# youssefg7/dl-sound-classification

Measured on AMD Instinct MI355X. Metric: training clips/sec (EnvNet-v2, ESC-50 shape), higher is better.
Workload: dtype bf16; 1 GPU; EnvNet-v2 train step (BC-mix, fwd, soft-CE, bwd, clip, Adam), ESC-50 shape; global_batch=256, per_gpu_batch=256, clip_samples=220500, parallelism=dp1, model=envnet_v2

## Files before the change

### dl-sound-classification_amd/csrc/feconv.hip

```cpp
#include "common.h"

#include <type_traits>

namespace {

constexpr int F1_DEPTH = 4;
constexpr int FE_NT = 256;
constexpr int FE_BM = 128;
constexpr int FE_N = 64;

typedef unsigned u32x4 __attribute__((ext_vector_type(4)));

template <int CIN, int KW, int S>
struct FeCfg {
  static constexpr int CG = CIN / 8;
  static constexpr int WPX = (FE_BM - 1) * S + KW;
  static constexpr int HALF = (WPX + 1) / 2;
  static constexpr int NSLOT = S == 1 ? WPX : 2 * HALF;
  static constexpr int PSB = CIN * 2 + 16;
  static constexpr int WBYTES = NSLOT * PSB;
  static constexpr int NCH = WPX * CG;
  static constexpr int LCH = (NCH + FE_NT - 1) / FE_NT;
  static constexpr int KS = KW * CIN / 16;
  static_assert(FE_NT % CG == 0, "channel chunk must be constant per thread");
  static_assert(KS == 32, "weights-in-registers layout assumes K = 512");
};

struct FeArgs {
  const bf16* x;
  const float* ps;
  const float* pt;
  const bf16* w;
  const float* bias;
// ... 180 lines not shown
    if (blockIdx.x < 64 && kst < 256 && lane == 0) {
#pragma unroll
      for (int k = 0; k < 8; ++k) g_fe_st[(((int)blockIdx.x * 4 + wave) * 256 + kst) * 8 + k] = ts[k];
    }
    ++kst;
#endif
  };

  int item = blockIdx.x;
  load(item, rawa, oka);
  load(item + (int)gridDim.x, rawb, okb);
  __syncthreads();
  store(0, rawa, oka);
  __syncthreads();
  for (;;) {
    step(item, 0, rawa, oka, rawb, okb);
    item += gridDim.x;
    if (item >= items) break;
    step(item, 1, rawb, okb, rawa, oka);
    item += gridDim.x;
    if (item >= items) break;
  }
}

constexpr int FS_NT = 512;
#ifndef FS_DEPTH
#define FS_DEPTH 3
#endif
#ifndef FS_FD
#define FS_FD 4
#endif


template <int CIN, int KW, int S, bool PRE>
__global__ __launch_bounds__(FS_NT) __attribute__((amdgpu_waves_per_eu(2, 2))) void feconv_ws_kernel(FeArgs g) {
  using Cfg = FeCfg<CIN, KW, S>;
  __shared__ __attribute__((aligned(16))) char smem[2 * Cfg::WBYTES];
  __shared__ __attribute__((aligned(16))) float sbias[FE_N];
  __shared__ __attribute__((aligned(16))) float spre[2][CIN];
  const int t = threadIdx.x, lane = t & 63, wave = t >> 6;
  const int items = g.n * g.nitem;
  if ((int)blockIdx.x >= items) return;
  const int nk = (items - 1 - (int)blockIdx.x) / (int)gridDim.x + 1;
  if (t < FE_N) sbias[t] = g.bias ? g.bias[t] : 0.f;
  if (PRE && t < CIN) {
    spre[0][t] = g.ps[t];
    spre[1][t] = g.pt[t];
  }
  if (wave < 4) {
    const int nh = wave & 1, pq = wave >> 1;
    bf16x8 wf[Cfg::KS];
    {
      const bf16* wr = g.w + (int64_t)(nh * 32 + (lane & 31)) * (KW * CIN) + 8 * (lane >> 5);
#pragma unroll
      for (int ks = 0; ks < Cfg::KS; ++ks) wf[ks] = *reinterpret_cast<const bf16x8*>(wr + ks * 16);
    }
    const int c0 = nh * 32 + 8 * (lane >> 5);
    lds_barrier();
    lds_barrier();
#pragma unroll 1
    for (int k = 0; k < nk; ++k) {
      const int item = (int)blockIdx.x + k * (int)gridDim.x;
      f32x16 acc[2];
#pragma unroll
      for (int i = 0; i < 2; ++i)
#pragma unroll
        for (int r = 0; r < 16; ++r) acc[i][r] = 0.f;
      const char* win = smem + (k & 1) * Cfg::WBYTES;
      auto frag = [&](int ks, int i) __attribute__((always_inline)) {
        constexpr int KPC = CIN / 16;
        const int kx = ks / KPC;
        const int ci = (ks % KPC) * 16 + 8 * (lane >> 5);
        const int px = pq * 64 + i * 32 + (lane & 31);
        int slot;
        if constexpr (S == 1) slot = px + kx;
        else slot = (kx & 1) * Cfg::HALF + px + (kx >> 1);
        return *reinterpret_cast<const bf16x8*>(win + slot * Cfg::PSB + ci * 2);
      };
#ifdef FS_PROBE_NOCOMPUTE
      if (g.n < 0)
#endif
      {
        bf16x8 fr[FS_FD][2];
#pragma unroll
        for (int ks = 0; ks < FS_FD; ++ks)
#pragma unroll
          for (int i = 0; i < 2; ++i) fr[ks][i] = frag(ks, i);
#pragma unroll
        for (int ks = 0; ks < Cfg::KS; ++ks) {
#pragma unroll
          for (int i = 0; i < 2; ++i) {
            acc[i] = __builtin_amdgcn_mfma_f32_32x32x16_bf16(wf[ks], fr[ks % FS_FD][i], acc[i], 0, 0, 0);
            if (ks + FS_FD < Cfg::KS) fr[ks % FS_FD][i] = frag(ks + FS_FD, i);
          }
        }
        __builtin_amdgcn_sched_group_barrier(0x100, 2 * FS_FD, 0);
#pragma unroll
        for (int ks = 0; ks < Cfg::KS; ++ks) {
          __builtin_amdgcn_sched_group_barrier(0x008, 2, 0);
          if (ks + FS_FD < Cfg::KS) __builtin_amdgcn_sched_group_barrier(0x100, 2, 0);
        }
      }
      const int b = item / g.nitem;
      const int m0 = (item - b * g.nitem) * FE_BM + pq * 64;
      bf16* yb = g.y + (int64_t)b * g.ystride;
#pragma unroll
      for (int i = 0; i < 2; ++i) {
        float v[16];
#pragma unroll
        for (int h = 0; h < 2; ++h)
#pragma unroll
          for (int j = 0; j < 4; ++j) {
            const float lo = acc[i][8 * h + j], hi = acc[i][8 * h + 4 + j];
            const auto r = __builtin_amdgcn_permlane32_swap(__float_as_uint(lo), __float_as_uint(hi), false, false);
            v[8 * h + j] = __builtin_bit_cast(float, (unsigned)r[0]);
            v[8 * h + 4 + j] = __builtin_bit_cast(float, (unsigned)r[1]);
          }
        const int m = m0 + i * 32 + (lane & 31);
        if (m < g.wout) {
#pragma unroll
          for (int h = 0; h < 2; ++h) {
            const int64_t e = (int64_t)m * FE_N + c0 + 16 * h;
            if (e < g.ylen) {
              const f32x4 u0 = *reinterpret_cast<const f32x4*>(sbias + c0 + 16 * h);
              const f32x4 u1 = *reinterpret_cast<const f32x4*>(sbias + c0 + 16 * h + 4);
              const u32x4 o = {pack2(v[8 * h] + u0[0], v[8 * h + 1] + u0[1]), pack2(v[8 * h + 2] + u0[2], v[8 * h + 3] + u0[3]),
                               pack2(v[8 * h + 4] + u1[0], v[8 * h + 5] + u1[1]), pack2(v[8 * h + 6] + u1[2], v[8 * h + 7] + u1[3])};
              *reinterpret_cast<u32x4*>(yb + e) = o;
            }
          }
        }
      }
      lds_barrier();
    }
  } else {
    const int ft = t - 256;
    const int cg = ft % Cfg::CG;
    const __amdgpu_buffer_rsrc_t xr = __builtin_amdgcn_make_buffer_rsrc(
        const_cast<bf16*>(g.x), (short)0, (int)((int64_t)g.n * g.win * CIN * 2), 0x00020000);
    auto load = [&](int k, u32x4 (&raw)[Cfg::LCH], uint32_t& rok) __attribute__((always_inline)) {
      int it = (int)blockIdx.x + k * (int)gridDim.x;
      it = it < items ? it : items - 1;
      const int b = it / g.nitem;
      const int px0 = (it - b * g.nitem) * FE_BM * S - g.pw;
      rok = 0;
#pragma unroll
      for (int s = 0; s < Cfg::LCH; ++s) {
        const int q = ft + FE_NT * s;
        const int p = q / Cfg::CG;
        const int ix = px0 + p;
        const bool ok = p < Cfg::WPX && ix >= 0 && ix < g.win;
        const unsigned off = ok ? (unsigned)((b * g.win + ix) * Cfg::CG + cg) * 16u : 0x80000000u;
#ifdef FS_PROBE_NOLOAD
        raw[s] = u32x4{0u, 0u, 0u, 0u};
        (void)off;
#else
        raw[s] = __builtin_bit_cast(u32x4, __builtin_amdgcn_raw_buffer_load_b128(xr, off, 0, 0));
#endif
        rok |= (uint32_t)ok << s;
      }
    };
    auto stage = [&](int buf, const u32x4 (&raw)[Cfg::LCH], uint32_t rok) __attribute__((always_inline)) {
      float sc[8], sh[8];
      if constexpr (PRE) {
#pragma unroll
        for (int h = 0; h < 2; ++h) {
// ... 12 lines not shown
              fe_cook(raw[s], (rok >> s) & 1u, PRE, sc, sh);
      }
    };
    u32x4 raw[FS_DEPTH][Cfg::LCH];
    uint32_t rok[FS_DEPTH];
#pragma unroll
    for (int d = 0; d < FS_DEPTH; ++d) load(d, raw[d], rok[d]);
    lds_barrier();
    stage(0, raw[0], rok[0]);
    lds_barrier();
    static_assert(12 % FS_DEPTH == 0, "feeder unroll");
    auto iter = [&](auto KC, int k) __attribute__((always_inline)) {
      constexpr int R = decltype(KC)::value;
      constexpr int SET = R % FS_DEPTH, NXT = (R + 1) % FS_DEPTH;
      load(k + FS_DEPTH, raw[SET], rok[SET]);
      if (k + 1 < nk) stage((R + 1) & 1, raw[NXT], rok[NXT]);
      lds_barrier();
    };
    auto step = [&](auto KC, int k) __attribute__((always_inline)) {
      const int kk = k + decltype(KC)::value;
      if (kk < nk) iter(KC, kk);
      return kk + 1 < nk;
    };
#pragma unroll 1
    for (int k = 0; k < nk; k += 12) {
      using std::integral_constant;
      (void)(step(integral_constant<int, 0>{}, k) && step(integral_constant<int, 1>{}, k) &&
             step(integral_constant<int, 2>{}, k) && step(integral_constant<int, 3>{}, k) &&
             step(integral_constant<int, 4>{}, k) && step(integral_constant<int, 5>{}, k) &&
             step(integral_constant<int, 6>{}, k) && step(integral_constant<int, 7>{}, k) &&
             step(integral_constant<int, 8>{}, k) && step(integral_constant<int, 9>{}, k) &&
             step(integral_constant<int, 10>{}, k) && step(integral_constant<int, 11>{}, k));
    }
  }
}

struct F1Args {
  const float* x;
  const bf16* w;
  const float* bias;
  bf16* y;
  float* part;
  int n, t, w1, nitem;
};

template <bool STATS>
__global__ __launch_bounds__(256) void fe_conv1_kernel(F1Args g) {
  __shared__ __attribute__((aligned(16))) uint32_t seg[4][160];
  __shared__ __attribute__((aligned(16))) char stage[4][2048];
  const int lane = threadIdx.x & 63, wv = threadIdx.x >> 6;
  const int gw = blockIdx.x * 4 + wv, nw = gridDim.x * 4;
  const int items = g.n * g.nitem;
  uint32_t* sg = seg[wv];
  bf16x8 wa[4];
#pragma unroll
  for (int ks = 0; ks < 4; ++ks) wa[ks] = *reinterpret_cast<const bf16x8*>(g.w + (lane & 31) * 64 + ks * 16 + 8 * (lane >> 5));
  const int c0 = 8 * (lane >> 5);
  float bv[16];
#pragma unroll
  for (int i = 0; i < 8; ++i) { bv[i] = g.bias[c0 + i]; bv[8 + i] = g.bias[c0 + 16 + i]; }
  float s1[16], s2[16];
#pragma unroll
  for (int i = 0; i < 16; ++i) { s1[i] = 0.f; s2[i] = 0.f; }

  typedef float f32x2 __attribute__((ext_vector_type(2)));
  auto load = [&](int it) __attribute__((always_inline)) {
// ... 512 lines not shown
bool reduce_v1() { const char* e = getenv("MIA_REDUCE_V1"); return e && e[0] == '1'; }

bool aligned16(const void* p) { return (reinterpret_cast<uintptr_t>(p) & 15) == 0; }

bool fe_ws() { const char* e = getenv("MIA_FECONV_WS"); return !(e && e[0] == '0'); }

}

extern "C" int mia_fe_conv2_fwd(const void* y1, const float* scale, const float* shift, const void* w,
                                const float* bias, void* y2, int32_t n, int32_t w1, int32_t w2,
                                mia_stream_t stream) {
  MIA_CHECK_ARG(y1 && w && y2 && n > 0 && w1 >= 16, "fe_conv2_fwd: bad arguments");
  MIA_CHECK_ARG(!scale == !shift, "fe_conv2_fwd: scale and shift go together");
  MIA_CHECK_ARG(w2 == (w1 - 16) / 2 + 1, "fe_conv2_fwd: w2 must be (w1-16)/2+1 (got w1=%d w2=%d)", w1, w2);
  MIA_CHECK_ARG(aligned16(y1) && aligned16(w) && aligned16(y2), "fe_conv2_fwd: operands must be 16-byte aligned");
  hipStream_t s = as_stream(stream);
  const int per = fe_clips_per_launch((int64_t)w1 * 32 * 2);
  MIA_CHECK_ARG(per > 0, "fe_conv2_fwd: one clip exceeds 2 GB");
  for (int c = 0; c < n; c += per) {
    const int nc = n - c < per ? n - c : per;
    FeArgs a{reinterpret_cast<const bf16*>(y1) + (int64_t)c * w1 * 32, scale, shift, reinterpret_cast<const bf16*>(w),
             bias, reinterpret_cast<bf16*>(y2) + (int64_t)c * w2 * FE_N, nc, w1, w2, 0, (int)cdiv(w2, FE_BM),
             (int64_t)w2 * FE_N, (int64_t)w2 * FE_N};
    if (fe_ws()) {
      const int grid = fe_grid1(nc * a.nitem);
      if (scale) feconv_ws_kernel<32, 16, 2, true><<<grid, FS_NT, 0, s>>>(a);
      else feconv_ws_kernel<32, 16, 2, false><<<grid, FS_NT, 0, s>>>(a);
    } else {
      const int grid = fe_grid(nc * a.nitem);
      if (scale) feconv_kernel<32, 16, 2, true><<<grid, FE_NT, 0, s>>>(a);
      else feconv_kernel<32, 16, 2, false><<<grid, FE_NT, 0, s>>>(a);
    }
    MIA_LAUNCH_CHECK("fe_conv2_fwd");
  }
  return 0;
}

extern "C" int mia_fe_conv2_dgrad(const void* dy2, const void* wpar, void* da1, int32_t n, int32_t w1,
                                  int32_t w2, mia_stream_t stream) {
  MIA_CHECK_ARG(dy2 && wpar && da1 && n > 0 && w1 >= 16, "fe_conv2_dgrad: bad arguments");
  MIA_CHECK_ARG(w2 == (w1 - 16) / 2 + 1, "fe_conv2_dgrad: w2 must be (w1-16)/2+1 (got w1=%d w2=%d)", w1, w2);
  MIA_CHECK_ARG(aligned16(dy2) && aligned16(wpar) && aligned16(da1), "fe_conv2_dgrad: operands must be 16-byte aligned");
  MIA_CHECK_ARG(((int64_t)w1 * 32) % 8 == 0, "fe_conv2_dgrad: clip stride must keep 16-byte alignment");
  const int wout = (w1 + 1) / 2;
  const int per = fe_clips_per_launch((int64_t)w2 * 64 * 2);
  MIA_CHECK_ARG(per > 0, "fe_conv2_dgrad: one clip exceeds 2 GB");
  for (int c = 0; c < n; c += per) {
    const int nc = n - c < per ? n - c : per;
    FeArgs a{reinterpret_cast<const bf16*>(dy2) + (int64_t)c * w2 * 64, nullptr, nullptr,
             reinterpret_cast<const bf16*>(wpar), nullptr, reinterpret_cast<bf16*>(da1) + (int64_t)c * w1 * 32, nc,
             w2, wout, 7, (int)cdiv(wout, FE_BM), (int64_t)w1 * 32, (int64_t)w1 * 32};
#ifdef FS_DGRAD
    feconv_ws_kernel<64, 8, 1, false><<<fe_grid1(nc * a.nitem), FS_NT, 0, as_stream(stream)>>>(a);
#else
    feconv_kernel<64, 8, 1, false><<<fe_grid(nc * a.nitem), FE_NT, 0, as_stream(stream)>>>(a);
#endif
    MIA_LAUNCH_CHECK("fe_conv2_dgrad");
  }
  return 0;
}

extern "C" int mia_fe_conv2_wgrad(const void* dy2, const void* y1, const float* scale, const float* shift,
                                  float* dw, int32_t n, int32_t w1, int32_t w2, void* workspace, int64_t ws_bytes,
                                  mia_stream_t stream) {
  MIA_CHECK_ARG(dy2 && y1 && dw && workspace && n > 0 && w1 >= 16, "fe_conv2_wgrad: bad arguments");
  MIA_CHECK_ARG(!scale == !shift, "fe_conv2_wgrad: scale and shift go together");
// ... 65 lines not shown
```

### dl-sound-classification_amd/src/miaudio/kernels.py

```python
from __future__ import annotations

import math
from dataclasses import dataclass

import os

import torch

from . import lib as L

_WS: dict = {}


def workspace(nbytes: int, device, slot: str = "main") -> torch.Tensor:
    key = (str(device), slot)
    buf = _WS.get(key)
    nbytes = max(int(nbytes), 256)
    if buf is None or buf.numel() < nbytes:
        buf = torch.empty(int(nbytes * 1.25) + 256, dtype=torch.uint8, device=device)
        _WS[key] = buf
    return buf


def _s():
# ... 463 lines not shown
    assert dw.dtype == torch.float32 and dw.numel() == 32 * 64 and dbias.dtype == torch.float32 and dbias.numel() == 32
    nw = 4096
    lib = L.load()
    part = workspace(int(lib.mia_conv3_wgrad_workspace_bytes(nw)), x.device, "conv3w")
    with probe(tag or "", 2.0 * n * oh * ow * 32 * 64, x.numel() * 2 + da.numel() * 6):
        L.check(lib.mia_conv3_wgrad_bn(x.data_ptr(), da.data_ptr(), ya.data_ptr(), dy.data_ptr(), dw.data_ptr(),
                                       dbias.data_ptr(), part.data_ptr(), nw, n, h, wd, L.ptr(gamma),
                                       bn.scale.data_ptr(), bn.shift.data_ptr(), bn.mean.data_ptr(),
                                       bn.invstd.data_ptr(), dgamma.data_ptr(), dbeta.data_ptr(), _s()),
                "mia_conv3_wgrad_bn")


def bn_finalize_shifted(partial: torch.Tensor, nblk: int, P: int, C: int, kshift: torch.Tensor, gamma, beta,
                        running_mean, running_var, momentum: float, eps: float) -> BNState:
    st = torch.empty(4, C, dtype=torch.float32, device=partial.device)
    L.check(L.load().mia_bn_finalize_shifted(partial.data_ptr(), nblk, P, C, kshift.data_ptr(), L.ptr(gamma),
                                             L.ptr(beta), L.ptr(running_mean), L.ptr(running_var), momentum, eps, 1,
                                             st[0].data_ptr(), st[1].data_ptr(), st[2].data_ptr(), st[3].data_ptr(),
                                             _s()), "mia_bn_finalize_shifted")
    return BNState(st[0], st[1], st[2], st[3])


def fe_conv2_fwd(y1: torch.Tensor, scale, shift, w: torch.Tensor, bias, y2: torch.Tensor, n: int, w1: int,
                 w2: int, tag: str | None = None):
    assert y1.dtype == torch.bfloat16 and y2.dtype == torch.bfloat16 and w.dtype == torch.bfloat16
    assert y1.numel() == n * w1 * 32 and y2.numel() == n * w2 * 64 and w.numel() == 64 * 512
    assert y1.is_contiguous() and y2.is_contiguous() and w.is_contiguous()
    flop = 2.0 * n * w2 * 64 * 512
    with probe(tag or "", flop, y1.numel() * 2 + y2.numel() * 2):
        L.check(L.load().mia_fe_conv2_fwd(y1.data_ptr(), L.ptr(scale), L.ptr(shift), w.data_ptr(), L.ptr(bias),
                                          y2.data_ptr(), n, w1, w2, _s()), "mia_fe_conv2_fwd")


def fe_conv2_dgrad(dy2: torch.Tensor, wpar: torch.Tensor, da1: torch.Tensor, n: int, w1: int, w2: int,
                   tag: str | None = None):
    assert dy2.dtype == torch.bfloat16 and da1.dtype == torch.bfloat16 and wpar.dtype == torch.bfloat16
    assert dy2.numel() == n * w2 * 64 and da1.numel() == n * w1 * 32 and wpar.numel() == 64 * 512
    assert dy2.is_contiguous() and da1.is_contiguous() and wpar.is_contiguous()
    flop = 2.0 * n * w1 * 32 * 512
    with probe(tag or "", flop, dy2.numel() * 2 + da1.numel() * 2):
        L.check(L.load().mia_fe_conv2_dgrad(dy2.data_ptr(), wpar.data_ptr(), da1.data_ptr(), n, w1, w2, _s()),
                "mia_fe_conv2_dgrad")


def fe_conv2_wgrad(dy2: torch.Tensor, y1: torch.Tensor, scale, shift, dw: torch.Tensor, n: int, w1: int, w2: int,
                   tag: str | None = None):
    assert dy2.dtype == torch.bfloat16 and y1.dtype == torch.bfloat16 and dw.dtype == torch.float32
    assert dy2.numel() == n * w2 * 64 and y1.numel() == n * w1 * 32 and dw.numel() == 64 * 512
    nlaunch = -(-(n * w1 * 64) // (2 ** 31 - 1)) + 1
    nbytes = 512 * nlaunch * 64 * 512 * 4
    ws = workspace(nbytes, dy2.device, "fw")
    flop = 2.0 * n * w2 * 64 * 512
    with probe(tag or "", flop, (dy2.numel() + y1.numel()) * 2):
        L.check(L.load().mia_fe_conv2_wgrad(dy2.data_ptr(), y1.data_ptr(), L.ptr(scale), L.ptr(shift), dw.data_ptr(),
                                            n, w1, w2, ws.data_ptr(), ws.numel(), _s()), "mia_fe_conv2_wgrad")


def fe_conv1_wgrad_bn(x: torch.Tensor, dact: torch.Tensor, y1: torch.Tensor, n: int, t: int, gamma, bn: BNState,
                      dw: torch.Tensor, dbias: torch.Tensor, tag: str | None = None):
    w1 = (t - 64) // 2 + 1
    assert dact.dtype == torch.bfloat16 and y1.dtype == torch.bfloat16 and x.dtype == torch.float32
    assert dact.numel() == n * w1 * 32 and y1.numel() == n * w1 * 32 and x.numel() == n * t
    assert dw.numel() == 32 * 64 and dw.dtype == torch.float32 and dbias.numel() == 32
    split = 512
    ws = workspace((split * (2 * 2048 + 96) + 2 * 2048 + n * 80 + 2 * 160 + 4) * 4, x.device, "tapw")
    g = torch.empty(2, 32, dtype=torch.float32, device=x.device)
# ... 379 lines not shown
```

### dl-sound-classification_amd/src/miaudio/lib.py

```python
from __future__ import annotations

import ctypes as C
import os
from pathlib import Path

import torch

PKG_ROOT = Path(__file__).resolve().parents[2]
LIB_PATH = Path(os.environ.get("MIAUDIO_LIB") or PKG_ROOT / "lib" / "libmiaudio.so")

F32, BF16, U8 = 0, 1, 2
MXFP8 = 16
OP_DENSE, OP_CONV, OP_CONVROW = 0, 1, 2
KC, RC = 0, 1
PRE_NONE, PRE_AFFINE, PRE_AFFINE_RELU, PRE_GELU = 0, 1, 2, 3
ACT_NONE, ACT_RELU, ACT_GELU, DACT_NZ, DACT_GELU, ACT_ADD_AUX, ACT_GELU_SAVE = 0, 1, 2, 3, 4, 5, 6
ACT_GELU_SAVE_D, DACT_MUL = 7, 8

vp = C.c_void_p
i32 = C.c_int32
i64 = C.c_int64
f32 = C.c_float


# ... 118 lines not shown
    "mia_tokens_bwd": (C.c_int, [vp, vp, vp, vp, i32, i32, i32, vp]),
    "mia_ast_patches": (C.c_int, [vp, i32, i32, i32, i32, i32, vp, vp]),
    "mia_tokens_fwd_inplace": (C.c_int, [vp, vp, vp, i32, i32, i32, vp]),
    "mia_cast": (C.c_int, [vp, i32, vp, i32, i64, vp]),
    "mia_add_inplace": (C.c_int, [vp, vp, i32, i64, vp]),
    "mia_bc_mix": (C.c_int, [vp, vp, i64, i32, vp, vp, vp, vp, i32, vp, vp, vp, vp, vp]),
    "mia_bc_partner": (C.c_int, [vp, i32, vp, i32, vp, vp, vp]),
    "mia_stretch_gain": (C.c_int, [vp, i64, i32, vp, vp, vp, vp]),
    "mia_spec_augment_mixup":(C.c_int, [vp, vp, vp, i32, i32, i32, vp, vp, vp, vp, vp, vp, vp]),
    "mia_leaf_workspace_bytes": (i64, [i32, i64, i32, i32, i32, i32]),
    "mia_leaf_energy_fwd": (C.c_int, [vp, vp, vp, i32, i64, i32, i32, i32, i32, vp, vp]),
    "mia_leaf_energy_bwd": (C.c_int, [vp, vp, vp, vp, i32, i64, i32, i32, i32, i32, vp, vp]),
    "mia_pcen_workspace_bytes": (i64, [i32, i32]),
    "mia_pcen_fwd": (C.c_int, [vp, vp, vp, f32, vp, i32, i32, i32, vp]),
    "mia_pcen_bwd": (C.c_int, [vp, vp, vp, f32, vp, vp, vp, vp, vp, i32, i32, i32, vp]),
    "mia_lt_stats_blocks": (i32, [i32, i32, i32, i32]),
    "mia_lt_workspace_bytes": (i64, [i32]),
    "mia_lt_pool_stats": (C.c_int, [vp, i32, i32, i32, i32, i32, vp, vp, vp, vp, vp, i32, vp]),
    "mia_lt_pool_apply": (C.c_int, [vp, i32, i32, i32, i32, vp, vp, vp, i32, i32, vp]),
    "mia_lt_pool_bwd_gather": (C.c_int, [vp, i32, i32, vp, i32, i32, i32, i32, vp, vp, vp, vp, vp, vp, vp, vp, vp]),
    "mia_lt_pool_bwd_apply": (C.c_int, [vp, vp, vp, i32, i32, i32, i32, i32, vp, vp, vp, vp, vp, vp, vp, vp, vp]),
    "mia_lt_pcen_fwd": (C.c_int, [vp, vp, vp, f32, vp, i32, i32, i32, i32, i32, vp]),
    "mia_lt_pcen_bwd": (C.c_int, [vp, vp, vp, f32, vp, i32, vp, vp, vp, vp, i32, i32, i32, i32, vp]),
    "mia_resample_out_len": (i64, [i64, i32, i32]),
    "mia_resample": (C.c_int, [vp, i64, i32, i64, vp, vp, i32, i32, i32, vp, i64, i64, vp]),
    "mia_clip_sgd": (C.c_int, [vp, vp, vp, vp, vp, i32, i64, i64, f32, f32, f32, f32, i32, f32, vp, vp, vp, vp, vp,
                               vp]),
    "mia_clip_adamw": (C.c_int, [vp, vp, vp, vp, vp, vp, i32, i64, i64, f32, f32, f32, f32, f32, i32, f32, vp, vp, vp,
                                 vp, vp, vp]),
    "mia_gemm_sgd": (C.c_int, [P(MiaOperand), P(MiaOperand), i64, i64, i64, vp, vp, vp, i64, vp, f32, f32, f32, f32,
                               i32, i32, vp]),
    "mia_gemm_adamw": (C.c_int, [P(MiaOperand), P(MiaOperand), i64, i64, i64, vp, vp, vp, vp, i64, vp, f32, f32, f32,
                                 f32, f32, f32, f32, vp]),
    "mia_last_error_string": (C.c_char_p, []),
    "mia_device_arch": (C.c_int, [C.c_char_p, i32]),
}

_LIB = None


def load(path: Path | str | None = None):
    global _LIB
    if _LIB is not None:
        return _LIB
    p = Path(path) if path else LIB_PATH
    if not p.exists():
        raise RuntimeError(f"libmiaudio.so not found at {p}: build it with `make -C {PKG_ROOT}` "
                           "(the MI355X kernels have no CPU fallback)")
    lib = C.CDLL(str(p))
    for name, (res, args) in SIGNATURES.items():
        fn = getattr(lib, name, None)
        if fn is None:
            continue
        fn.restype = res
        fn.argtypes = args
    _LIB = lib
    return lib


def exported_symbols():
    lib = load()
    return {n for n in SIGNATURES if hasattr(lib, n)}


def check(rc: int, what: str):
    if rc != 0:
# ... 37 lines not shown
```

### dl-sound-classification_amd/src/models/envnet_hip.py

```python
from __future__ import annotations

import itertools
import os

import torch

from ..miaudio import kernels as K
from ..miaudio import lib as L

_SEED = itertools.count(0x5EED)
C8_BNSEP = os.environ.get("MIA_C8_BNSEP", "0") == "1"
C3_BNSEP = os.environ.get("MIA_C3_BNSEP", "0") == "1"
FC1_CHUNK_ROWS = 256


def _use_conv8(cd: int, cin: int, cout: int, kh: int, kw: int) -> bool:
    return cd == L.BF16 and cin == 32 and cout == 32 and kh == 8 and kw == 8

TRUNK = [
    (("trunk", 0, 0), ("trunk", 0, 1), 1, 32, 8, 8),
    (("trunk", 0, 3), ("trunk", 0, 4), 32, 32, 8, 8),
    (("trunk", 1, 0), ("trunk", 1, 1), 32, 64, 1, 4),
    (("trunk", 1, 3), ("trunk", 1, 4), 64, 64, 1, 4),
    (("trunk", 2, 0), ("trunk", 2, 1), 64, 128, 1, 2),
    (("trunk", 2, 3), ("trunk", 2, 4), 128, 128, 1, 2),
    (("trunk", 3, 0), ("trunk", 3, 1), 128, 256, 1, 2),
    (("trunk", 3, 3), ("trunk", 3, 4), 256, 256, 1, 2),
]
TRUNK_POOL = [(5, 3), (1, 2), (1, 2), (1, 2)]


def geometry(T: int):
    W1 = (T - 64) // 2 + 1
    W2 = (W1 - 16) // 2 + 1
    Wp = W2 // 64
    g = {"T": T, "W1": W1, "W2": W2, "Wp": Wp, "trunk": []}
    H, W = 64, Wp
    for blk in range(4):
        ka = TRUNK[2 * blk]
        ha, wa = H - ka[4] + 1, W - ka[5] + 1
        kb = TRUNK[2 * blk + 1]
        hb, wb = ha - kb[4] + 1, wa - kb[5] + 1
        ph, pw = TRUNK_POOL[blk]
        g["trunk"].append(((H, W), (ha, wa), (hb, wb), (hb // ph, wb // pw)))
        H, W = hb // ph, wb // pw
    g["flat"] = 256 * H * W
    return g


def _frontend_work(B: int, g: dict, tdt: torch.dtype, backward: bool):
    es = torch.finfo(tdt).bits // 8
    X = g["T"] * 4
    S1 = g["W1"] * 32 * es
    S2 = g["W2"] * 64 * es
    P = 64 * g["Wp"] * es
    flop = 2.0 * (g["W1"] * 32 * 64 + g["W2"] * 64 * 512)
    if backward:
        return B * 2 * flop, B * (P + 4 * S2 + 4 * S1 + X)
    return B * flop, B * (X + 2 * S1 + 2 * S2 + P)


def _param_list(m):
    ps = [m.frontend[0].weight, m.frontend[0].bias, m.frontend[1].weight, m.frontend[1].bias,
          m.frontend[3].weight, m.frontend[3].bias, m.frontend[4].weight, m.frontend[4].bias]
    for blk in range(4):
        seq = m.trunk[blk]
        ps += [seq[0].weight, seq[0].bias, seq[1].weight, seq[1].bias,
               seq[3].weight, seq[3].bias, seq[4].weight, seq[4].bias]
    for idx in (1, 4, 7):
        ps += [m.classifier[idx].weight, m.classifier[idx].bias]
    return ps


def _bns(m):
    out = [m.frontend[1], m.frontend[4]]
    for blk in range(4):
        out += [m.trunk[blk][1], m.trunk[blk][4]]
    return out


class EnvNetFunction(torch.autograd.Function):
    @staticmethod
    def forward(ctx, model, x, compute: int, *params):
        if not x.is_cuda:
            raise RuntimeError("EnvNetV2 runs on the MI355X HIP kernels only (input is on CPU)")
        B = x.shape[0]
        x = x.reshape(B, -1).contiguous().float()
        T = x.shape[1]
        if T % 2:
            raise ValueError(f"EnvNetV2 expects an even clip length (got {T})")
        g = geometry(T)
        if g["flat"] != model.classifier[1].in_features:
            raise ValueError(f"clip length {T} gives {g['flat']} trunk features, FC1 expects "
                             f"{model.classifier[1].in_features} (envnet_v2.py:51)")
        training = model.training
        cd = compute
        tdt = L.torch_dtype(cd)
        dev = x.device
        bns = _bns(model)
        p = params
        W1, W2, Wp = g["W1"], g["W2"], g["Wp"]
        saved = {"g": g, "B": B, "cd": cd}

        def bn(i, y, P, C):
            mod = bns[i]
            return K.bn_fwd_stats(y, P, C, mod.weight, mod.bias, mod.running_mean, mod.running_var,
                                  mod.momentum if mod.momentum is not None else 0.1, mod.eps, training)

        wpk = dict(zip([0, 4] + [8 + 8 * b + o for b in range(4) for o in (0, 4)],
                       K.pack_weights([(p[i], cd, 0) for i in [0, 4] + [8 + 8 * b + o for b in range(4) for o in (0, 4)]])))
        saved["wpk"] = wpk
        fe = K.probe("frontend.fwd", *_frontend_work(B, g, tdt, backward=False))
        fe.__enter__()
        w1 = wpk[0]
        y1 = torch.empty(B * W1, 32, dtype=tdt, device=dev)
        if cd == L.BF16:
            st = K.fe_conv1_fwd(x, w1, p[1], y1, B, T, stats=training, tag="conv1.fwd")
            if training:
                m0 = bns[0]
                bn1 = K.bn_finalize_shifted(st[0], st[1], B * W1, 32, p[1], m0.weight, m0.bias, m0.running_mean,
                                            m0.running_var, m0.momentum if m0.momentum is not None else 0.1, m0.eps)
            else:
                bn1 = bn(0, y1, B * W1, 32)
        else:
            A = K.conv(x, L.KC, B, 1, T // 2, 2, 1, W1, 1, 32, row_kind=True)
            Bo = K.dense(w1, L.KC, 32, 64)
            K.gemm(A, Bo, K.epilogue(y1, 32, bias=p[1]), B * W1, 32, 64, cd, tag="conv1.fwd")
            bn1 = bn(0, y1, B * W1, 32)
        w2 = wpk[4]
        y2 = torch.empty(B * W2, 64, dtype=tdt, device=dev)
        if cd == L.BF16:
            K.fe_conv2_fwd(y1, bn1.scale, bn1.shift, w2, p[5], y2, B, W1, W2, tag="conv2.fwd")
        else:
            A = K.conv(y1, L.KC, B, 1, W1, 32, 1, W2, 1, 16, sw=2, pre=L.PRE_AFFINE_RELU, scale=bn1.scale,
                       shift=bn1.shift)
            K.gemm(A, K.dense(w2, L.KC, 64, 512), K.epilogue(y2, 64, bias=p[5]), B * W2, 64, 512, cd,
                   tag="conv2.fwd")
        X0 = torch.empty(B, 64, Wp, dtype=tdt, device=dev)
        am0 = torch.empty(B, Wp, 64, dtype=torch.uint8, device=dev)
        if cd == L.BF16 and training:
            win0 = torch.empty(B, Wp, 64, dtype=tdt, device=dev)
            part2, nb2 = K.pool_raw_stats(y2, B, 1, W2, 64, 1, 64, p[6], p[5], win0, am0)
            m1 = bns[1]
            bn2 = K.bn_finalize_shifted(part2, nb2, B * W2, 64, p[5], m1.weight, m1.bias, m1.running_mean,
                                        m1.running_var, m1.momentum if m1.momentum is not None else 0.1, m1.eps)
            K.pool_apply(win0, B, 1, Wp, 64, bn2, X0, 1)
        else:
            bn2 = bn(1, y2, B * W2, 64)
            K.pool_fwd(y2, B, 1, W2, 64, 1, 64, bn2, X0, 1, am0)
        fe.__exit__(None, None, None)
        saved.update(x=x, y1=y1, y2=y2, bn1=bn1, bn2=bn2, X0=X0, am0=am0,
                     win0=win0 if cd == L.BF16 and training else None)

        inp = X0
        trunk_saved = []
        for blk in range(4):
            (H, W), (ha, wa), (hb, wb), (hp, wp) = g["trunk"][blk]
            _, _, cin, cout, kh, kw = TRUNK[2 * blk]
            pa = 8 + 8 * blk
            wa_ = wpk[pa]
            ya = torch.empty(B * ha * wa, cout, dtype=tdt, device=dev)
            dense_w2 = cd == L.BF16 and kh == 1 and kw == 2 and cin > 1
            conv3_st = None
            if dense_w2:
                K.conv_w2_fwd(inp.reshape(B * H * W, cin), B * H, W, cin, wa_, p[pa + 1], ya, tag=f"t{blk}a.fwd")
            elif cd == L.BF16 and cin == 1 and kh == 8 and kw == 8 and cout == 32 and W % 4 == 0:
                conv3_st = K.fe_conv3_fwd(inp, wa_, p[pa + 1], ya, B, H, W, stats=training, tag=f"t{blk}a.fwd")
            else:
                if cin == 1:
                    A = K.conv(inp, L.KC, B, H, W, 1, ha, wa, kh, kw, row_kind=True)
                else:
                    A = K.conv(inp, L.KC, B, H, W, cin, ha, wa, kh, kw)
                K.gemm(A, K.dense(wa_, L.KC, cout, kh * kw * cin), K.epilogue(ya, cout, bias=p[pa + 1]),
                       B * ha * wa, cout, kh * kw * cin, cd, tag=f"t{blk}a.fwd")
            if conv3_st is not None:
# ... 302 lines not shown
```

Before: 15260 clips/s.

## Fuse BN statistics and max-pool window selection into conv2 forward epilogue

Adds a POOL variant of the warp-specialized conv2 kernel whose epilogue computes per-channel shifted BN sum/sumsq partials and the sign-aware argmax over each 64-wide pool window, writing the pooled raw value and argmax index directly. The training frontend path uses it by default, skipping the separate pool_raw_stats pass that re-read the conv2 output. In exchange the epilogue gains cross-lane permutes, DPP reductions, an extra barrier and a final LDS reduction, which raises register pressure in a kernel pinned to two waves per EU.

```diff
diff --git a/dl-sound-classification_amd/csrc/feconv.hip b/dl-sound-classification_amd/csrc/feconv.hip
--- a/dl-sound-classification_amd/csrc/feconv.hip
+++ b/dl-sound-classification_amd/csrc/feconv.hip
@@ -1,4 +1,6 @@
 #include "common.h"
+
+#include "../../include/miaudio_frontend.h"
 
 #include <type_traits>
 
@@ -245,12 +247,37 @@
 #endif
 
 
-template <int CIN, int KW, int S, bool PRE>
-__global__ __launch_bounds__(FS_NT) __attribute__((amdgpu_waves_per_eu(2, 2))) void feconv_ws_kernel(FeArgs g) {
+struct FePoolArgs : FeArgs {
+  const float* gamma;
+  uint16_t* pwin;
+  uint8_t* amax;
+  float* part;
+  int wp, slot0, zfrom, nslots;
+};
+
+typedef float f32x2 __attribute__((ext_vector_type(2)));
+typedef short s16x2 __attribute__((ext_vector_type(2)));
+
+__device__ __forceinline__ uint32_t fe_code2(uint32_t k) {
+  const s16x2 a = __builtin_bit_cast(s16x2, k) >> (short)15;
+  const s16x2 x = __builtin_bit_cast(s16x2, k & 0x7fff7fffu) ^ a;
+  return __builtin_bit_cast(uint32_t, (s16x2)(x - a));
+}
+template <int N>
+__device__ __forceinline__ int fe_max_ror(int v) {
+  const int o = __builtin_amdgcn_update_dpp(0, v, 0x120 + N, 0xf, 0xf, true);
+  return o > v ? o : v;
+}
+
+template <int CIN, int KW, int S, bool PRE, bool POOL = false>
+__global__ __launch_bounds__(FS_NT) __attribute__((amdgpu_waves_per_eu(2, 2))) void feconv_ws_kernel(
+    std::conditional_t<POOL, FePoolArgs, FeArgs> g) {
   using Cfg = FeCfg<CIN, KW, S>;
   __shared__ __attribute__((aligned(16))) char smem[2 * Cfg::WBYTES];
   __shared__ __attribute__((aligned(16))) float sbias[FE_N];
   __shared__ __attribute__((aligned(16))) float spre[2][CIN];
+  __shared__ __attribute__((aligned(16))) uint32_t ssgn[FE_N / 2];
+  static_assert(!POOL || 4 * 64 * 33 * 4 <= 2 * Cfg::WBYTES, "statistics image fits the window buffers");
   const int t = threadIdx.x, lane = t & 63, wave = t >> 6;
   const int items = g.n * g.nitem;
   if ((int)blockIdx.x >= items) return;
@@ -260,6 +287,9 @@
     spre[0][t] = g.ps[t];
     spre[1][t] = g.pt[t];
   }
+  if constexpr (POOL) {
+    if (t < FE_N / 2) ssgn[t] = (g.gamma[2 * t] < 0.f ? 0x8000u : 0u) | (g.gamma[2 * t + 1] < 0.f ? 0x80000000u : 0u);
+  }
   if (wave < 4) {
     const int nh = wave & 1, pq = wave >> 1;
     bf16x8 wf[Cfg::KS];
@@ -269,6 +299,19 @@
       for (int ks = 0; ks < Cfg::KS; ++ks) wf[ks] = *reinterpret_cast<const bf16x8*>(wr + ks * 16);
     }
     const int c0 = nh * 32 + 8 * (lane >> 5);
+    const int cb = nh * 32 + 4 * (lane >> 5);
+    const int lch = cb + 2 * (lane & 1) + ((lane >> 4) & 1) + 8 * ((lane >> 1) & 3);
+    const int posf = 63 - (lane & 31);
+    uint32_t lsgn = 0;
+    bool lgz = false;
+    f32x2 s1[8], s2[8];
+    if constexpr (POOL) {
+      const float gv = g.gamma[lch];
+      lsgn = gv < 0.f ? 0x8000u : 0u;
+      lgz = gv == 0.f;
+#pragma unroll
+      for (int pp = 0; pp < 8; ++pp) s1[pp] = s2[pp] = f32x2{0.f, 0.f};
+    }
     lds_barrier();
     lds_barrier();
 #pragma unroll 1
@@ -317,6 +360,102 @@
       const int b = item / g.nitem;
       const int m0 = (item - b * g.nitem) * FE_BM + pq * 64;
       bf16* yb = g.y + (int64_t)b * g.ystride;
+      if constexpr (POOL) {
+#ifndef FS_POOL_LATE_BARRIER
+        lds_barrier();
+#endif
+        float bv[16];
+        uint32_t sg[8];
+#pragma unroll
+        for (int q = 0; q < 4; ++q) {
+          const f32x4 u = *reinterpret_cast<const f32x4*>(sbias + cb + 8 * q);
+          const uint2 m2 = *reinterpret_cast<const uint2*>(ssgn + (cb >> 1) + 4 * q);
+#pragma unroll
+          for (int j = 0; j < 4; ++j) bv[4 * q + j] = u[j];
+          sg[2 * q] = m2.x;
+          sg[2 * q + 1] = m2.y;
+        }
+        uint32_t P[2][8];
+#pragma unroll
+        for (int i = 0; i < 2; ++i)
+#pragma unroll
+          for (int pp = 0; pp < 8; ++pp)
+            P[i][pp] = pack2(acc[i][2 * pp] + bv[2 * pp], acc[i][2 * pp + 1] + bv[2 * pp + 1]);
+        const bool full = m0 + 64 <= g.wout;
+        auto stats = [&](auto MASKED) __attribute__((always_inline)) {
+#pragma unroll
+          for (int i = 0; i < 2; ++i) {
+            const bool ok = m0 + i * 32 + (lane & 31) < g.wout;
+#pragma unroll
+            for (int pp = 0; pp < 8; ++pp) {
+              const f32x2 f = {__uint_as_float(P[i][pp] << 16), __uint_as_float(P[i][pp] & 0xffff0000u)};
+              f32x2 d = f - f32x2{bv[2 * pp], bv[2 * pp + 1]};
+              if constexpr (decltype(MASKED)::value) d = ok ? d : f32x2{0.f, 0.f};
+              s1[pp] += d;
+              s2[pp] = __builtin_elementwise_fma(d, d, s2[pp]);
+            }
+          }
+        };
+        if (full) {
+          stats(std::false_type{});
+          int R[8];
+#pragma unroll
+          for (int pp = 0; pp < 8; ++pp) {
+            const uint32_t c0 = fe_code2(P[0][pp] ^ sg[pp]), c1 = fe_code2(P[1][pp] ^ sg[pp]);
+            const int l0 = (int)((c0 << 16) | (uint32_t)posf), l1 = (int)((c1 << 16) | (uint32_t)(posf - 32));
+            const int h0 = (int)((c0 & 0xffff0000u) | (uint32_t)posf), h1 = (int)((c1 & 0xffff0000u) | (uint32_t)(posf - 32));
+            const int ka = l0 > l1 ? l0 : l1, kb = h0 > h1 ? h0 : h1;
+            const auto sw = __builtin_amdgcn_permlane16_swap((unsigned)ka, (unsigned)kb, false, false);
+            const int u0 = (int)sw[0], u1 = (int)sw[1];
+            R[pp] = u0 > u1 ? u0 : u1;
+          }
+#pragma unroll
+          for (int pp = 0; pp < 8; ++pp) R[pp] = fe_max_ror<1>(fe_max_ror<2>(fe_max_ror<4>(fe_max_ror<8>(R[pp]))));
+          int kk = R[0];
+#pragma unroll
+          for (int pp = 1; pp < 8; ++pp) kk = (lane & 7) == pp ? R[pp] : kk;
+          const int code = kk >> 16;
+          int pos = 63 - (kk & 0xffff);
+          uint32_t raw = (uint32_t)(code < 0 ? (-code) | 0x8000 : code) ^ lsgn;
+          const bool fix = code == 0 || lgz;
+          if (__builtin_amdgcn_ballot_w64(fix)) {
+            pos = lgz ? 0 : pos;
+            const int src = ((lane & 32) + (pos & 31)) * 4;
+            uint32_t got = 0;
+#pragma unroll
+            for (int pp = 0; pp < 8; ++pp) {
+              const uint32_t t0 = (uint32_t)__builtin_amdgcn_ds_bpermute(src, (int)P[0][pp]);
+              const uint32_t t1 = (uint32_t)__builtin_amdgcn_ds_bpermute(src, (int)P[1][pp]);
+              if ((lane & 7) == pp) got = pos & 32 ? t1 : t0;
+            }
+            got = lane & 16 ? got >> 16 : got & 0xffffu;
+            raw = fix ? got : raw;
+          }
+          if (!(lane & 8)) {
+            const int64_t o = ((int64_t)b * g.wp + (m0 >> 6)) * FE_N + lch;
+            g.pwin[o] = (uint16_t)raw;
+            g.amax[o] = (uint8_t)pos;
+          }
+        } else {
+          stats(std::true_type{});
+        }
+#pragma unroll
+        for (int i = 0; i < 2; ++i) {
+          const int m = m0 + i * 32 + (lane & 31);
+#pragma unroll
+          for (int h = 0; h < 2; ++h) {
+            const auto ra = __builtin_amdgcn_permlane32_swap(P[i][4 * h], P[i][4 * h + 2], false, false);
+            const auto rb = __builtin_amdgcn_permlane32_swap(P[i][4 * h + 1], P[i][4 * h + 3], false, false);
+            const int64_t e = (int64_t)m * FE_N + c0 + 16 * h;
+            if (m < g.wout && e < g.ylen)
+              *reinterpret_cast<u32x4*>(yb + e) = u32x4{(unsigned)ra[0], (unsigned)rb[0], (unsigned)ra[1], (unsigned)rb[1]};
+          }
+        }
+#ifdef FS_POOL_LATE_BARRIER
+        lds_barrier();
+#endif
+        continue;
+      }
 #pragma unroll
       for (int i = 0; i < 2; ++i) {
         float v[16];
@@ -345,6 +484,23 @@
         }
       }
       lds_barrier();
+    }
+    if constexpr (POOL) {
+      float* red = reinterpret_cast<float*>(smem) + wave * (64 * 33);
+#pragma unroll
+      for (int pp = 0; pp < 8; ++pp) {
+        red[lane * 33 + 2 * pp] = s1[pp][0];
+        red[lane * 33 + 2 * pp + 1] = s1[pp][1];
+        red[lane * 33 + 16 + 2 * pp] = s2[pp][0];
+        red[lane * 33 + 16 + 2 * pp + 1] = s2[pp][1];
+      }
+      wave_sync();
+      const int v = lane & 31, r = v & 15;
+      float a = 0.f;
+#pragma unroll 8
+      for (int p = 0; p < 32; ++p) a += red[((lane & 32) + p) * 33 + v];
+      const int slot = g.slot0 + 2 * (int)blockIdx.x + pq;
+      g.part[((int64_t)slot * FE_N + cb + (r & 3) + 8 * (r >> 2)) * 2 + (v >> 4)] = a;
     }
   } else {
     const int ft = t - 256;
@@ -423,6 +579,10 @@
              step(integral_constant<int, 8>{}, k) && step(integral_constant<int, 9>{}, k) &&
              step(integral_constant<int, 10>{}, k) && step(integral_constant<int, 11>{}, k));
     }
+    if constexpr (POOL) {
+      if (blockIdx.x == 0)
+        for (int64_t e = (int64_t)g.zfrom * (FE_N * 2) + ft; e < (int64_t)g.nslots * (FE_N * 2); e += 256) g.part[e] = 0.f;
+    }
   }
 }
 
@@ -1001,6 +1161,58 @@
       else feconv_kernel<32, 16, 2, false><<<grid, FE_NT, 0, s>>>(a);
     }
     MIA_LAUNCH_CHECK("fe_conv2_fwd");
+  }
+  return 0;
+}
+
+extern "C" int32_t mia_fe_conv2_pool_slots(int32_t n, int32_t w1) {
+  if (n <= 0 || w1 < 16) return 0;
+  const int per = fe_clips_per_launch((int64_t)w1 * 32 * 2);
+  if (per <= 0) return 0;
+  const int nitem = (int)cdiv((w1 - 16) / 2 + 1, FE_BM);
+  int64_t slots = 0;
+  for (int c = 0; c < n; c += per) slots += 2 * fe_grid1((n - c < per ? n - c : per) * nitem);
+  return slots < (1ll << 31) ? (int32_t)slots : 0;
+}
+
+extern "C" int mia_fe_conv2_fwd_pool(const void* y1, const float* scale, const float* shift, const void* w,
+                                     const float* bias, void* y2, int32_t n, int32_t w1, int32_t w2,
+                                     const float* gamma, void* win, void* argmax, float* partial, int32_t nslots,
+                                     mia_stream_t stream) {
+  MIA_CHECK_ARG(y1 && w && y2 && n > 0 && w1 >= 16, "fe_conv2_fwd_pool: bad arguments");
+  MIA_CHECK_ARG(bias && gamma && partial && (w2 < 64 || (win && argmax)), "fe_conv2_fwd_pool: null pointer");
+  MIA_CHECK_ARG(!scale == !shift, "fe_conv2_fwd_pool: scale and shift go together");
+  MIA_CHECK_ARG(w2 == (w1 - 16) / 2 + 1, "fe_conv2_fwd_pool: w2 must be (w1-16)/2+1 (got w1=%d w2=%d)", w1, w2);
+  MIA_CHECK_ARG(aligned16(y1) && aligned16(w) && aligned16(y2), "fe_conv2_fwd_pool: operands must be 16-byte aligned");
+  MIA_CHECK_ARG((reinterpret_cast<uintptr_t>(win) & 1) == 0 && (reinterpret_cast<uintptr_t>(partial) & 3) == 0,
+                "fe_conv2_fwd_pool: win must be 2-byte and partial 4-byte aligned");
+  hipStream_t s = as_stream(stream);
+  const int per = fe_clips_per_launch((int64_t)w1 * 32 * 2);
+  MIA_CHECK_ARG(per > 0, "fe_conv2_fwd_pool: one clip exceeds 2 GB");
+  const int need = mia_fe_conv2_pool_slots(n, w1);
+  MIA_CHECK_ARG(need > 0 && nslots >= need, "fe_conv2_fwd_pool: %d partial slots given, %d needed", nslots, need);
+  const int wp = w2 / 64;
+  int slot0 = 0;
+  for (int c = 0; c < n; c += per) {
+    const int nc = n - c < per ? n - c : per;
+    FePoolArgs a;
+    static_cast<FeArgs&>(a) = FeArgs{reinterpret_cast<const bf16*>(y1) + (int64_t)c * w1 * 32, scale, shift,
+                                     reinterpret_cast<const bf16*>(w), bias,
+                                     reinterpret_cast<bf16*>(y2) + (int64_t)c * w2 * FE_N, nc, w1, w2, 0,
+                                     (int)cdiv(w2, FE_BM), (int64_t)w2 * FE_N, (int64_t)w2 * FE_N};
+    a.gamma = gamma;
+    a.pwin = reinterpret_cast<uint16_t*>(win) + (int64_t)c * wp * FE_N;
+    a.amax = reinterpret_cast<uint8_t*>(argmax) + (int64_t)c * wp * FE_N;
+    a.part = partial;
+    a.wp = wp;
+    a.slot0 = slot0;
+    a.zfrom = c == 0 ? need : nslots;
+    a.nslots = nslots;
+    const int grid = fe_grid1(nc * a.nitem);
+    if (scale) feconv_ws_kernel<32, 16, 2, true, true><<<grid, FS_NT, 0, s>>>(a);
+    else feconv_ws_kernel<32, 16, 2, false, true><<<grid, FS_NT, 0, s>>>(a);
+    MIA_LAUNCH_CHECK("fe_conv2_fwd_pool");
+    slot0 += 2 * grid;
   }
   return 0;
 }
diff --git a/dl-sound-classification_amd/src/miaudio/kernels.py b/dl-sound-classification_amd/src/miaudio/kernels.py
--- a/dl-sound-classification_amd/src/miaudio/kernels.py
+++ b/dl-sound-classification_amd/src/miaudio/kernels.py
@@ -519,6 +519,31 @@
                                           y2.data_ptr(), n, w1, w2, _s()), "mia_fe_conv2_fwd")
 
 
+def fe_conv2_pool_sizes(n: int, w2: int, nslots: int) -> dict:
+    wp = w2 // 64
+    return {"y2": n * w2 * 64 * 2, "win": n * wp * 64 * 2, "argmax": n * wp * 64, "partial": nslots * 64 * 2 * 4}
+
+
+def fe_conv2_fwd_pool(y1: torch.Tensor, scale, shift, w: torch.Tensor, bias: torch.Tensor, y2: torch.Tensor, n: int,
+                      w1: int, w2: int, gamma: torch.Tensor, win: torch.Tensor, argmax: torch.Tensor,
+                      tag: str | None = None):
+    assert y1.dtype == torch.bfloat16 and y2.dtype == torch.bfloat16 and w.dtype == torch.bfloat16
+    assert y1.numel() == n * w1 * 32 and y2.numel() == n * w2 * 64 and w.numel() == 64 * 512
+    assert y1.is_contiguous() and y2.is_contiguous() and w.is_contiguous()
+    assert win.dtype == torch.bfloat16 and argmax.dtype == torch.uint8 and gamma.dtype == torch.float32
+    assert win.numel() == n * (w2 // 64) * 64 and argmax.numel() == win.numel() and gamma.numel() == 64
+    assert win.is_contiguous() and argmax.is_contiguous() and bias is not None and bias.numel() == 64
+    lib = L.load()
+    nslots = int(lib.mia_fe_conv2_pool_slots(n, w1))
+    part = torch.empty(nslots, 64, 2, dtype=torch.float32, device=y1.device)
+    flop = 2.0 * n * w2 * 64 * 512
+    with probe(tag or "", flop, y1.numel() * 2 + y2.numel() * 2):
+        L.check(lib.mia_fe_conv2_fwd_pool(y1.data_ptr(), L.ptr(scale), L.ptr(shift), w.data_ptr(), bias.data_ptr(),
+                                          y2.data_ptr(), n, w1, w2, gamma.data_ptr(), win.data_ptr(),
+                                          argmax.data_ptr(), part.data_ptr(), nslots, _s()), "mia_fe_conv2_fwd_pool")
+    return part, nslots
+
+
 def fe_conv2_dgrad(dy2: torch.Tensor, wpar: torch.Tensor, da1: torch.Tensor, n: int, w1: int, w2: int,
                    tag: str | None = None):
     assert dy2.dtype == torch.bfloat16 and da1.dtype == torch.bfloat16 and wpar.dtype == torch.bfloat16
diff --git a/dl-sound-classification_amd/src/miaudio/lib.py b/dl-sound-classification_amd/src/miaudio/lib.py
--- a/dl-sound-classification_amd/src/miaudio/lib.py
+++ b/dl-sound-classification_amd/src/miaudio/lib.py
@@ -174,6 +174,8 @@
                                i32, i32, vp]),
     "mia_gemm_adamw": (C.c_int, [P(MiaOperand), P(MiaOperand), i64, i64, i64, vp, vp, vp, vp, i64, vp, f32, f32, f32,
                                  f32, f32, f32, f32, vp]),
+    "mia_fe_conv2_pool_slots": (i32, [i32, i32]),
+    "mia_fe_conv2_fwd_pool": (C.c_int, [vp, vp, vp, vp, vp, vp, i32, i32, i32, vp, vp, vp, vp, i32, vp]),
     "mia_last_error_string": (C.c_char_p, []),
     "mia_device_arch": (C.c_int, [C.c_char_p, i32]),
 }
diff --git a/dl-sound-classification_amd/src/models/envnet_hip.py b/dl-sound-classification_amd/src/models/envnet_hip.py
--- a/dl-sound-classification_amd/src/models/envnet_hip.py
+++ b/dl-sound-classification_amd/src/models/envnet_hip.py
@@ -48,7 +48,11 @@
     return g
 
 
-def _frontend_work(B: int, g: dict, tdt: torch.dtype, backward: bool):
+def _fe_conv2_pool() -> bool:
+    return os.environ.get("MIA_FECONV_POOL", "1") != "0" and os.environ.get("MIA_FECONV_WS", "1") != "0"
+
+
+def _frontend_work(B: int, g: dict, tdt: torch.dtype, backward: bool, fused_pool: bool = False):
     es = torch.finfo(tdt).bits // 8
     X = g["T"] * 4
     S1 = g["W1"] * 32 * es
@@ -57,7 +61,7 @@
     flop = 2.0 * (g["W1"] * 32 * 64 + g["W2"] * 64 * 512)
     if backward:
         return B * 2 * flop, B * (P + 4 * S2 + 4 * S1 + X)
-    return B * flop, B * (X + 2 * S1 + 2 * S2 + P)
+    return B * flop, B * (X + 2 * S1 + (1 if fused_pool else 2) * S2 + P)
 
 
 def _param_list(m):
@@ -110,7 +114,8 @@
         wpk = dict(zip([0, 4] + [8 + 8 * b + o for b in range(4) for o in (0, 4)],
                        K.pack_weights([(p[i], cd, 0) for i in [0, 4] + [8 + 8 * b + o for b in range(4) for o in (0, 4)]])))
         saved["wpk"] = wpk
-        fe = K.probe("frontend.fwd", *_frontend_work(B, g, tdt, backward=False))
+        fused_pool = cd == L.BF16 and training and _fe_conv2_pool()
+        fe = K.probe("frontend.fwd", *_frontend_work(B, g, tdt, backward=False, fused_pool=fused_pool))
         fe.__enter__()
         w1 = wpk[0]
         y1 = torch.empty(B * W1, 32, dtype=tdt, device=dev)
@@ -129,7 +134,12 @@
             bn1 = bn(0, y1, B * W1, 32)
         w2 = wpk[4]
         y2 = torch.empty(B * W2, 64, dtype=tdt, device=dev)
-        if cd == L.BF16:
+        am0 = torch.empty(B, Wp, 64, dtype=torch.uint8, device=dev)
+        if fused_pool:
+            win0 = torch.empty(B, Wp, 64, dtype=tdt, device=dev)
+            part2, nb2 = K.fe_conv2_fwd_pool(y1, bn1.scale, bn1.shift, w2, p[5], y2, B, W1, W2, p[6], win0, am0,
+                                             tag="conv2.fwd")
+        elif cd == L.BF16:
             K.fe_conv2_fwd(y1, bn1.scale, bn1.shift, w2, p[5], y2, B, W1, W2, tag="conv2.fwd")
         else:
             A = K.conv(y1, L.KC, B, 1, W1, 32, 1, W2, 1, 16, sw=2, pre=L.PRE_AFFINE_RELU, scale=bn1.scale,
@@ -137,10 +147,10 @@
             K.gemm(A, K.dense(w2, L.KC, 64, 512), K.epilogue(y2, 64, bias=p[5]), B * W2, 64, 512, cd,
                    tag="conv2.fwd")
         X0 = torch.empty(B, 64, Wp, dtype=tdt, device=dev)
-        am0 = torch.empty(B, Wp, 64, dtype=torch.uint8, device=dev)
         if cd == L.BF16 and training:
-            win0 = torch.empty(B, Wp, 64, dtype=tdt, device=dev)
-            part2, nb2 = K.pool_raw_stats(y2, B, 1, W2, 64, 1, 64, p[6], p[5], win0, am0)
+            if not fused_pool:
+                win0 = torch.empty(B, Wp, 64, dtype=tdt, device=dev)
+                part2, nb2 = K.pool_raw_stats(y2, B, 1, W2, 64, 1, 64, p[6], p[5], win0, am0)
             m1 = bns[1]
             bn2 = K.bn_finalize_shifted(part2, nb2, B * W2, 64, p[5], m1.weight, m1.bias, m1.running_mean,
                                         m1.running_var, m1.momentum if m1.momentum is not None else 0.1, m1.eps)
diff --git a/include/miaudio_frontend.h b/include/miaudio_frontend.h
--- /dev/null
+++ b/include/miaudio_frontend.h
@@ -0,0 +1,21 @@
+#ifndef MIAUDIO_FRONTEND_H
+#define MIAUDIO_FRONTEND_H
+#include "miaudio.h"
+
+#ifdef __cplusplus
+extern "C" {
+#endif
+
+#define MIA_FE_POOL_KW 64
+
+int32_t mia_fe_conv2_pool_slots(int32_t n, int32_t w1);
+
+int mia_fe_conv2_fwd_pool(const void* y1, const float* scale, const float* shift, const void* w,
+                          const float* bias, void* y2, int32_t n, int32_t w1, int32_t w2,
+                          const float* gamma, void* win, void* argmax, float* partial, int32_t nslots,
+                          mia_stream_t stream);
+
+#ifdef __cplusplus
+}
+#endif
+#endif
```

Measured after the change: 15410 clips/s (median of 6 runs). About the same (+0.9%).
